# ktncktnc/diffusion-forcing-transformer

Hardware: AMD Instinct MI355X
Metric: denoised latent frames/sec, DFoT RE10K 8f & 200f rollout @1/2/4/8 GPU (higher is better)
Workload: dtype bf16

## Files before the change

### diffusion-forcing-transformer_amd/csrc/gemm.h

```cpp
#pragma once
#include "common.h"

namespace dfot {

enum AMode { A_DENSE = 0, A_CONV3 = 1, A_CONV3T = 2 };
enum Epi { E_F32 = 0, E_BF16 = 1, E_QKV = 2, E_QKV_DIT = 3 };

struct GemmArgs {
  const bf16* A = nullptr;
  long lda = 0;
  const bf16* W = nullptr;
  long ldw = 0;
  int M = 0, N = 0, K = 0;
  int H = 0, Wd = 0, Cin = 0;
  const bf16* zeros = nullptr;
  const uint8_t* live = nullptr;
  int To = 0, Tin = 0, Hin = 0, Win = 0;
  int cs = 1, ct = 1, ckt = 1;
  const float* bias = nullptr;
  float* out_f32 = nullptr;
  bf16* out_bf16 = nullptr;
  long ldo = 0;
  const float* resid = nullptr;
  const bf16* resid_bf = nullptr;
  const float* gate = nullptr;
  const int* gate_index = nullptr;
  long ldg = 0;
  int gate_rows = 0;
  int act = 0;
  bf16* pre_act = nullptr;
  bf16* raw = nullptr;
  long ldraw = 0;
  int bias_rows = 0;
  int tr_rows = 0;
  float* gn_part = nullptr;
  int gn_rows_per_bt = 0;
  int gn_cpg = 0;
  bf16* out2 = nullptr;
  long ldo2 = 0;
  int split = 0;
  bf16 *q = nullptr, *k = nullptr, *v = nullptr;
  const float *qw = nullptr, *kw = nullptr, *rope_cs = nullptr;
  int heads = 0, d = 0, ntok = 0;
  float qscale = 1.f;
  int dstride = 0;
  float eps = 1e-6f;
  int xcd = 1;
  int persist = 0;
  int ksplit = 1;
  long slice_stride = 0;
};

enum GemmVariant {
  GEMM_REGS_128 = 0,
  GEMM_DMA_128 = 1,
  GEMM_DMA_256x256 = 4,
  GEMM_DMA_512x128 = 6,
  GEMM_DMA_128_KS2 = 8,
  GEMM_DMA_256x192 = 9,
  GEMM_DMA_128x192 = 10,
  GEMM_DMA3_256x144 = 14,
  GEMM_AUTO = -1
};
int gemm_pick_variant(int amode, int m, int n, int k, bool plain_f32 = false);
int launch_gemm(int amode, int epi, int variant, const GemmArgs& g, hipStream_t stream);

}
```

### diffusion-forcing-transformer_amd/csrc/gemm.hip

```cpp
#include "gemm.h"
#include "dfot_hip.h"

namespace dfot {

constexpr int BK = 64;
constexpr int wave_cols(int bn) { return bn % 64 == 0 ? 64 : 48; }
constexpr int tile_threads(int bm, int bn, int wtm, int ks) { return (bm / wtm) * (bn / wave_cols(bn)) * 64 * ks; }
constexpr int EP_LD = 68;

template <int N>
__device__ __forceinline__ void wait_all_but() {
  static_assert(N == 2 || N == 4 || N == 6 || N == 8 || N == 12, "unexpected load count");
  if constexpr (N == 2) asm volatile("s_waitcnt vmcnt(2)\n\ts_barrier" ::: "memory");
  if constexpr (N == 4) asm volatile("s_waitcnt vmcnt(4)\n\ts_barrier" ::: "memory");
  if constexpr (N == 6) asm volatile("s_waitcnt vmcnt(6)\n\ts_barrier" ::: "memory");
  if constexpr (N == 8) asm volatile("s_waitcnt vmcnt(8)\n\ts_barrier" ::: "memory");
  if constexpr (N == 12) asm volatile("s_waitcnt vmcnt(12)\n\ts_barrier" ::: "memory");
}

__device__ __forceinline__ void wait_all_but_n(int n) {
  switch (n) {
    case 1: asm volatile("s_waitcnt vmcnt(1)\n\ts_barrier" ::: "memory"); break;
    case 2: asm volatile("s_waitcnt vmcnt(2)\n\ts_barrier" ::: "memory"); break;
    case 3: asm volatile("s_waitcnt vmcnt(3)\n\ts_barrier" ::: "memory"); break;
    case 4: asm volatile("s_waitcnt vmcnt(4)\n\ts_barrier" ::: "memory"); break;
    case 5: asm volatile("s_waitcnt vmcnt(5)\n\ts_barrier" ::: "memory"); break;
    case 6: asm volatile("s_waitcnt vmcnt(6)\n\ts_barrier" ::: "memory"); break;
    case 7: asm volatile("s_waitcnt vmcnt(7)\n\ts_barrier" ::: "memory"); break;
    case 8: asm volatile("s_waitcnt vmcnt(8)\n\ts_barrier" ::: "memory"); break;
    default: asm volatile("s_waitcnt vmcnt(0)\n\ts_barrier" ::: "memory"); break;
  }
}

template <int BM_T, int BN_T, int WTM, int NST, int AMODE, int EPI, bool DMA, int KS, int BKT>
__device__ __forceinline__ void gemm_tile(const GemmArgs& g, const int tile_index, const int tile_count) {
  static_assert(BKT == 64 || (BKT == 32 && AMODE == A_DENSE && DMA && KS == 1), "K-tile depth");
  constexpr int CPR = BKT / 8;
  constexpr int RPI = 64 / CPR;
  constexpr int ROWB = BKT * 2;
  constexpr int MI = WTM / 16;
  constexpr int WTN = wave_cols(BN_T);
  constexpr int NI = WTN / 16;
  constexpr int WN = BN_T / WTN;
  static_assert(WTN == 64 || (EPI == E_F32 || EPI == E_BF16), "48-column wave tiles: plain epilogues only");
  static_assert(WTN == 64 || KS == 1, "48-column wave tiles: no intra-workgroup split-K");
  constexpr int NW = (BM_T / WTM) * WN;
  constexpr int NT = NW * 64;
  constexpr int AINS = BM_T / RPI, WINS = BN_T / RPI;
  constexpr int ACH = (AINS + NW - 1) / NW;
  constexpr int WCH = (WINS + NW - 1) / NW;
  constexpr bool A_EVEN = AINS % NW == 0, W_EVEN = WINS % NW == 0;
  static_assert((A_EVEN && W_EVEN) || (DMA && KS == 1), "uneven staging: LDS-DMA kernels without intra-workgroup split-K only");
  constexpr int A_BYTES = BM_T * BKT * 2;
  constexpr int STAGE_BYTES = (BM_T + BN_T) * BKT * 2;
  constexpr int LOADS = ACH + WCH;
  static_assert(DMA || NST == 2, "register staging supports two stages only");
  static_assert(KS == 1 || (NST == 2 && DMA && EPI != E_QKV), "split-K: two-stage LDS-DMA kernels without in-epilogue barriers");
  extern __shared__ __attribute__((aligned(16))) char smem_all[];
  const int tid = threadIdx.x, lane = tid & 63;
  const int kgroup = KS == 1 ? 0 : (tid >> 6) / NW;
  const int wave = KS == 1 ? (tid >> 6) : (tid >> 6) % NW;
  char* smem = smem_all + kgroup * (NST * STAGE_BYTES);
  const int wm = wave / WN, wn = wave % WN;
  const int tiles_n = (g.N + BN_T - 1) / BN_T;
  const int ksplit = (EPI == E_F32 && (AMODE == A_DENSE || g.slice_stride > 0) && g.ksplit > 1) ? g.ksplit : 1;
  const int kslice = ksplit > 1 ? tile_index % ksplit : 0;
  const int bid = ksplit > 1 ? xcd_remap(tile_index / ksplit, tile_count / ksplit, g.xcd) : xcd_remap(tile_index, tile_count, g.xcd);
  const int tn = bid % tiles_n, tm = bid / tiles_n;
  const int m0 = tm * BM_T, n0 = tn * BN_T;
  if constexpr (AMODE == A_CONV3) {
    if (g.live && !g.live[(unsigned)m0 / (unsigned)(g.H * g.Wd)]) return;
  }
  int nk = g.K / BKT;
  long kbeg = 0;
  if (ksplit > 1) {
    const int per = nk / ksplit, rem = nk % ksplit;
    kbeg = (long)(kslice * per + (kslice < rem ? kslice : rem)) * BKT;
    nk = per + (kslice < rem ? 1 : 0);
  }
  auto swz = [](int r) { return BKT == 64 ? ((r >> 1) & 7) : ((r >> 2) & 2); };

  const int prow = lane / CPR;
  const int ppos = lane % CPR;
  const bf16* a_src[ACH];
  int a_y[ACH], a_x[ACH];
  [[maybe_unused]] int a_t[ACH];
  const bf16* w_src[WCH];
  int a_chunk[ACH];
#pragma unroll
  for (int i = 0; i < ACH; ++i) {
    const int r = RPI * (NW * i + wave) + prow;
    const int c = ppos ^ swz(r);
    a_chunk[i] = c;
    const long m = (long)m0 + r;
    if constexpr (AMODE == A_DENSE) {
      a_src[i] = g.A + m * g.lda + c * 8 + kbeg;
      a_y[i] = a_x[i] = 0;
    } else if constexpr (AMODE == A_CONV3) {
      const unsigned mu = (unsigned)m;
      const int xw = (int)(mu % (unsigned)g.Wd);
      const int yh = (int)((mu / (unsigned)g.Wd) % (unsigned)g.H);
      a_x[i] = xw;
      a_y[i] = yh;
      a_src[i] = g.A + m * (long)g.Cin + c * 8;
    } else {
      unsigned mu = (unsigned)m;
      const int xo = (int)(mu % (unsigned)g.Wd);
      mu /= (unsigned)g.Wd;
      const int yo = (int)(mu % (unsigned)g.H);
      mu /= (unsigned)g.H;
// ... 24 lines not shown
    cv_dx = tap % 3 - 1;
  } else if constexpr (AMODE == A_CONV3T) {
    const int kbase = kgroup * BKT + (int)kbeg;
    const int tap = kbase / g.Cin;
    cv_c0 = kbase - tap * g.Cin;
    cv_dt = tap / 9;
    cv_dy = (tap % 9) / 3;
    cv_dx = tap % 3;
  }
  auto a_addr = [&](int i, int kt) -> const bf16* {
    if constexpr (AMODE == A_DENSE) {
      return a_src[i] + (long)kt * BKT;
    } else if constexpr (AMODE == A_CONV3) {
      const int yy = a_y[i] + cv_dy, xx = a_x[i] + cv_dx;
      const bool ok = (yy >= 0) && (yy < g.H) && (xx >= 0) && (xx < g.Wd);
      const bf16* p = a_src[i] + ((long)cv_dy * g.Wd + cv_dx) * g.Cin + cv_c0;
      return ok ? p : g.zeros + a_chunk[i] * 8;
    } else {
      int tt = a_t[i] + cv_dt;
      tt = tt < 0 ? 0 : tt;
      const int yy = a_y[i] + cv_dy, xx = a_x[i] + cv_dx;
      const bool ok = (yy >= 0) && (yy < g.Hin) && (xx >= 0) && (xx < g.Win);
      const bf16* p = a_src[i] + ((long)(tt * g.Hin + yy) * g.Win + xx) * g.Cin + cv_c0;
      return ok ? p : g.zeros + a_chunk[i] * 8;
    }
  };
  auto conv_advance = [&]() {
    if constexpr (AMODE == A_CONV3) {
      cv_c0 += KS * BKT;
      while (cv_c0 >= g.Cin) {
        cv_c0 -= g.Cin;
        if (++cv_dx > 1) {
          cv_dx = -1;
          ++cv_dy;
        }
      }
    } else if constexpr (AMODE == A_CONV3T) {
      cv_c0 += KS * BKT;
      while (cv_c0 >= g.Cin) {
        cv_c0 -= g.Cin;
        if (++cv_dx > 2) {
          cv_dx = 0;
          if (++cv_dy > 2) {
            cv_dy = 0;
            ++cv_dt;
          }
        }
      }
    }
  };

  bf16x8 ra[ACH], rw[WCH];

  auto issue = [&](int kt, int stage) {
    char* sa = smem + stage * STAGE_BYTES;
    char* sw = sa + A_BYTES;
#pragma unroll
    for (int i = 0; i < ACH; ++i) {
      if (!A_EVEN && NW * i + wave >= AINS) continue;
      const bf16* pa = a_addr(i, kt);
      if constexpr (DMA) {
        __builtin_amdgcn_global_load_lds(DFOT_GLOBAL_PTR(pa), DFOT_LDS_PTR(sa + (NW * i + wave) * 1024), 16, 0, 0);
      } else {
        ra[i] = *reinterpret_cast<const bf16x8*>(pa);
      }
    }
#pragma unroll
    for (int i = 0; i < WCH; ++i) {
      if (!W_EVEN && NW * i + wave >= WINS) continue;
      const bf16* pw = w_src[i] + (long)kt * BKT;
      if constexpr (DMA) {
        __builtin_amdgcn_global_load_lds(DFOT_GLOBAL_PTR(pw), DFOT_LDS_PTR(sw + (NW * i + wave) * 1024), 16, 0, 0);
      } else {
        rw[i] = *reinterpret_cast<const bf16x8*>(pw);
      }
    }
    conv_advance();
  };
  auto commit = [&](int stage) {
    char* sa = smem + stage * STAGE_BYTES;
    char* sw = sa + A_BYTES;
#pragma unroll
    for (int i = 0; i < ACH; ++i) *reinterpret_cast<bf16x8*>(sa + (NW * i + wave) * 1024 + lane * 16) = ra[i];
#pragma unroll
    for (int i = 0; i < WCH; ++i) *reinterpret_cast<bf16x8*>(sw + (NW * i + wave) * 1024 + lane * 16) = rw[i];
  };

  f32x4 acc[MI][NI];
#pragma unroll
  for (int i = 0; i < MI; ++i)
#pragma unroll
    for (int j = 0; j < NI; ++j) acc[i][j] = f32x4{0.f, 0.f, 0.f, 0.f};

  const int frow = lane & 15, fk = lane >> 4;
  auto compute = [&](int stage) {
    const char* sa = smem + stage * STAGE_BYTES;
    const char* sw = sa + A_BYTES;
#pragma unroll
    for (int ks = 0; ks < BKT / 32; ++ks) {
      bf16x8 af[MI], wf[NI];
#pragma unroll
      for (int mi = 0; mi < MI; ++mi) {
        const int r = wm * WTM + mi * 16 + frow;
        const int pos = (ks * 4 + fk) ^ swz(r);
        af[mi] = *reinterpret_cast<const bf16x8*>(sa + r * ROWB + pos * 16);
      }
#pragma unroll
      for (int ni = 0; ni < NI; ++ni) {
        const int r = wn * WTN + ni * 16 + frow;
        const int pos = (ks * 4 + fk) ^ swz(r);
        wf[ni] = *reinterpret_cast<const bf16x8*>(sw + r * ROWB + pos * 16);
      }
#pragma unroll
      for (int mi = 0; mi < MI; ++mi)
#pragma unroll
        for (int ni = 0; ni < NI; ++ni)
          acc[mi][ni] = __builtin_amdgcn_mfma_f32_16x16x32_bf16(af[mi], wf[ni], acc[mi][ni], 0, 0, 0);
    }
  };

  if constexpr (NST == 2 && KS == 1) {
    issue(0, 0);
    if constexpr (DMA) {
      asm volatile("s_waitcnt vmcnt(0)" ::: "memory");
    } else {
      commit(0);
    }
    __syncthreads();
    for (int kt = 0; kt < nk; ++kt) {
      const int cur = kt & 1;
      if (kt + 1 < nk) issue(kt + 1, cur ^ 1);
      compute(cur);
      if constexpr (DMA) {
        asm volatile("s_waitcnt vmcnt(0)" ::: "memory");
      } else {
        if (kt + 1 < nk) commit(cur ^ 1);
      }
      __syncthreads();
    }
  } else if constexpr (NST == 2) {
    const int nit = (nk + KS - 1) / KS;
    if (kgroup < nk) issue(kgroup, 0);
    asm volatile("s_waitcnt vmcnt(0)" ::: "memory");
    __syncthreads();
    for (int it = 0; it < nit; ++it) {
      const int cur = it & 1;
      const int kt = it * KS + kgroup;
      if (kt + KS < nk) issue(kt + KS, cur ^ 1);
      if (kt < nk) compute(cur);
      asm volatile("s_waitcnt vmcnt(0)" ::: "memory");
      __syncthreads();
    }
    float* red = reinterpret_cast<float*>(smem_all) + wave * (MI * 16 * 64);
    if (kgroup == 1) {
#pragma unroll
      for (int mi = 0; mi < MI; ++mi)
#pragma unroll
        for (int ni = 0; ni < 4; ++ni)
#pragma unroll
          for (int j = 0; j < 4; ++j) red[((mi * 4 + ni) * 4 + j) * 64 + lane] = acc[mi][ni][j];
    }
    __syncthreads();
    if (kgroup == 1) return;
#pragma unroll
    for (int mi = 0; mi < MI; ++mi)
#pragma unroll
      for (int ni = 0; ni < 4; ++ni)
#pragma unroll
        for (int j = 0; j < 4; ++j) acc[mi][ni][j] += red[((mi * 4 + ni) * 4 + j) * 64 + lane];
  } else {
    static_assert(NST >= 3, "ring");
    [[maybe_unused]] const int my_loads =
        __builtin_amdgcn_readfirstlane((AINS - wave + NW - 1) / NW + (WINS - wave + NW - 1) / NW);
    auto ring_wait = [&]() {
      if constexpr (A_EVEN && W_EVEN) wait_all_but<(NST - 2) * LOADS>();
      else wait_all_but_n((NST - 2) * my_loads);
    };
#pragma unroll
    for (int t = 0; t < NST - 1; ++t)
      if (t < nk) issue(t, t);
    if (nk >= NST - 1) {
      ring_wait();
    } else {
      asm volatile("s_waitcnt vmcnt(0)\n\ts_barrier" ::: "memory");
    }
    int st = 0;
    for (int kt = 0; kt < nk; ++kt) {
      const int nxt = st == 0 ? NST - 1 : st - 1;
      if (kt + NST - 1 < nk) issue(kt + NST - 1, nxt);
      compute(st);
      if (kt + NST - 1 < nk) {
        ring_wait();
      } else {
        asm volatile("s_waitcnt vmcnt(0)\n\ts_barrier" ::: "memory");
      }
      st = st == NST - 1 ? 0 : st + 1;
    }
  }

  float* ep =reinterpret_cast<float*>(smem_all) + (KS == 2 ? NW * MI * 16 * 64 : 0) + wave * (16 * EP_LD);
  const int colq = lane & 15, rowq = (lane >> 4) * 4;
  const int nw = n0 + wn * WTN;
  [[maybe_unused]] const bool has_res = g.resid != nullptr;
  [[maybe_unused]] const bool has_gate = g.gate != nullptr;
  [[maybe_unused]] float gsum = 0.f, gsq = 0.f, gsum2 = 0.f, gsq2 = 0.f;
  const int cw = EPI == E_F32 ? (lane & 15) * 4 : (lane & 7) * 8;
  const int col = nw + cw;
  const bool live = col < g.N && cw < WTN;
  f32x4 b0 = {0.f, 0.f, 0.f, 0.f}, b1 = {0.f, 0.f, 0.f, 0.f};
  [[maybe_unused]] const bool bias2d = g.bias_rows != 0;
  [[maybe_unused]] const unsigned bias_den = (unsigned)(g.bias_rows > 0 ? g.bias_rows : -g.bias_rows);
  [[maybe_unused]] const bool bias_mod = g.bias_rows > 0;
  [[maybe_unused]] float bc[NI];
  if constexpr (EPI == E_QKV) {
#pragma unroll
    for (int ni = 0; ni < NI; ++ni) {
      const int c = nw + ni * 16 + colq;
      bc[ni] = (g.bias && c < g.N) ? g.bias[c] : 0.f;
    }
  } else if (g.bias && live && !bias2d && kslice == 0) {
    b0 = *reinterpret_cast<const f32x4*>(g.bias + col);
    if constexpr (EPI != E_F32) b1 = *reinterpret_cast<const f32x4*>(g.bias + col + 4);
  }
  if constexpr (EPI == E_BF16) {
    if (g.tr_rows > 0) {
#pragma unroll
      for (int mi = 0; mi < MI; ++mi) {
        const unsigned row = (unsigned)(m0 + wm * WTM + mi * 16 + rowq);
        const long frame = row / (unsigned)g.tr_rows;
        const int rin = (int)(row % (unsigned)g.tr_rows);
#pragma unroll
        for (int ni = 0; ni < NI; ++ni) {
          const int c = nw + ni * 16 + colq;
          if (c < g.N) {
            bf16x4 o;
#pragma unroll
            for (int j = 0; j < 4; ++j) o[j] = f2bf(acc[mi][ni][j]);
            *reinterpret_cast<bf16x4*>(g.out_bf16 + (frame * g.N + c) * (long)g.tr_rows + rin) = o;
          }
        }
      }
      return;
    }
  }
  [[maybe_unused]] f32x4 res_cur[4], gate_cur;
  [[maybe_unused]] const bool pre_gate = EPI == E_F32 && has_gate && live && g.gate_rows % 16 == 0;
  [[maybe_unused]] auto load_gate = [&](int mi) {
    long gr = (unsigned)(m0 + wm * WTM + mi * 16) / (unsigned)g.gate_rows;
    if (g.gate_index) gr = g.gate_index[gr];
// ... 310 lines not shown
          }
        }
      }
    }
  }

  if constexpr (EPI == E_F32 || EPI == E_BF16) {
    if (g.gn_part) {
      const unsigned mrow = (unsigned)(m0 + wm * WTM);
      const int bt = (int)(mrow / (unsigned)g.gn_rows_per_bt);
      const int slots = g.gn_rows_per_bt / 64;
      const int slot = (int)((mrow % (unsigned)g.gn_rows_per_bt) / 64);
      float* dst = g.gn_part + ((long)bt * slots + slot) * 64;
      if constexpr (EPI == E_F32) {
        if (g.gn_cpg == 8) {
          gsum += __shfl_xor(gsum, 1);
          gsq += __shfl_xor(gsq, 1);
        }
        gsum += __shfl_xor(gsum, 16);
        gsq += __shfl_xor(gsq, 16);
        gsum += __shfl_xor(gsum, 32);
        gsq += __shfl_xor(gsq, 32);
        if (lane < 16 && live && (g.gn_cpg == 4 || (lane & 1) == 0)) {
          const int grp = col / g.gn_cpg;
          dst[grp * 2] = gsum;
          dst[grp * 2 + 1] = gsq;
        }
      } else {
        if (g.gn_cpg == 8) {
          gsum += gsum2;
          gsq += gsq2;
        }
#pragma unroll
        for (int o = 8; o < 64; o <<= 1) {
          gsum += __shfl_xor(gsum, o);
          gsq += __shfl_xor(gsq, o);
          gsum2 += __shfl_xor(gsum2, o);
          gsq2 += __shfl_xor(gsq2, o);
        }
        if (lane < 8 && live) {
          const int grp = col / g.gn_cpg;
          dst[grp * 2] = gsum;
          dst[grp * 2 + 1] = gsq;
          if (g.gn_cpg == 4) {
            dst[grp * 2 + 2] = gsum2;
            dst[grp * 2 + 3] = gsq2;
          }
        }
      }
    }
  }
}

template <int BM_T, int BN_T, int WTM, int NST, int AMODE, int EPI, bool DMA, int KS = 1, int BKT = BK>
__global__ __launch_bounds__(tile_threads(BM_T, BN_T, WTM, KS)) void gemm_kernel(GemmArgs g) {
  gemm_tile<BM_T, BN_T, WTM, NST, AMODE, EPI, DMA, KS, BKT>(g, blockIdx.x, gridDim.x);
}

template <int BM_T, int BN_T, int WTM, int NST, int AMODE, int EPI, bool DMA, int KS = 1, int BKT = BK>
__global__ __launch_bounds__(tile_threads(BM_T, BN_T, WTM, KS)) void gemm_kernel_persistent(GemmArgs g, int tile_count) {
  for (int tile = blockIdx.x; tile < tile_count; tile += gridDim.x) {
    gemm_tile<BM_T, BN_T, WTM, NST, AMODE, EPI, DMA, KS, BKT>(g, tile, tile_count);
    if (tile + (int)gridDim.x < tile_count) __syncthreads();
  }
}

template <int BM_T, int BN_T, int WTM, int NST, int AMODE, int EPI, bool DMA, int KS = 1, int BKT = BK>
static int launch_t(const GemmArgs& g, hipStream_t stream) {
  constexpr int nthreads = tile_threads(BM_T, BN_T, WTM, KS);
  constexpr int stage_lds = KS * NST * (BM_T + BN_T) * BKT * 2;
  constexpr int ep_lds = (nthreads / 64) * 16 * EP_LD * 4 + 2 * (nthreads / 64) * 16 * 4 +
                         (KS == 2 ? (nthreads / 128) * (WTM / 16) * 16 * 64 * 4 : 0);
  constexpr int lds = stage_lds > ep_lds ? stage_lds : ep_lds;
  const int ksplit = (EPI == E_F32 && (AMODE == A_DENSE || g.slice_stride > 0) && g.ksplit > 1) ? g.ksplit : 1;
  const int tiles = (g.M / BM_T) * ((g.N + BN_T - 1) / BN_T) * ksplit;
  GemmArgs ga = g;
  ga.xcd = 1;
  ga.persist = 1;
  constexpr bool kPersistOK = KS == 1 && nthreads <= 768;
  if constexpr (kPersistOK) {
    if (ga.persist > 0 && ksplit == 1) {
      const int resident = 256 * (lds <= 80 * 1024 ? 2 : 1);
      if (tiles > resident) {
        auto kp = gemm_kernel_persistent<BM_T, BN_T, WTM, NST, AMODE, EPI, DMA, KS, BKT>;
        static bool pattr_set = false;
        if (!pattr_set) {
          DFOT_CHECK_HIP(hipFuncSetAttribute(reinterpret_cast<const void*>(kp), hipFuncAttributeMaxDynamicSharedMemorySize, lds));
          pattr_set = true;
        }
        hipLaunchKernelGGL(kp, dim3(resident), dim3(nthreads), lds, stream, ga, tiles);
        DFOT_CHECK_HIP(hipGetLastError());
        return DFOT_OK;
      }
    }
  }
  auto kern = gemm_kernel<BM_T, BN_T, WTM, NST, AMODE, EPI, DMA, KS, BKT>;
  static bool attr_set = false;
  if (!attr_set) {
    DFOT_CHECK_HIP(hipFuncSetAttribute(reinterpret_cast<const void*>(kern), hipFuncAttributeMaxDynamicSharedMemorySize, lds));
    attr_set = true;
  }
  hipLaunchKernelGGL(kern, dim3(tiles), dim3(nthreads), lds, stream, ga);
  DFOT_CHECK_HIP(hipGetLastError());
  return DFOT_OK;
}

template <int AMODE, int EPI>
static int launch_v(int variant, const GemmArgs& g, hipStream_t s) {
  switch (variant) {
    case GEMM_REGS_128:
      if constexpr (AMODE == A_CONV3T) break;
      else return launch_t<128, 128, 64, 2, AMODE, EPI, false>(g, s);
    case GEMM_DMA_128: return launch_t<128, 128, 64, 2, AMODE, EPI, true>(g, s);
    case GEMM_DMA_256x256: return launch_t<256, 256, 64, 2, AMODE, EPI, true>(g, s);
    case GEMM_DMA_512x128: return launch_t<512, 128, 64, 2, AMODE, EPI, true>(g, s);
    case GEMM_DMA_256x192:
      if constexpr (AMODE != A_DENSE) break;
      else return launch_t<256, 192, 64, 2, AMODE, EPI, true>(g, s);
    case GEMM_DMA3_256x144:
      if constexpr ((EPI != E_F32 && !(EPI == E_BF16 && AMODE == A_DENSE)) || AMODE == A_CONV3T) break;
      else {
        if (g.gn_part) break;
        return launch_t<256, 144, 64, 3, AMODE, EPI, true>(g, s);
      }
    case GEMM_DMA_128x192:
      if constexpr (AMODE != A_DENSE || EPI == E_QKV) break;
      else return launch_t<128, 192, 64, 2, AMODE, EPI, true>(g, s);
    case GEMM_DMA_128_KS2:
      if constexpr (EPI == E_QKV) break;
      else return launch_t<128, 128, 64, 2, AMODE, EPI, true, 2>(g, s);
  }
  set_error("gemm: unknown variant %d", variant);
  return DFOT_ERR_ARG;
}

int gemm_pick_variant(int amode, int m, int n, int k, bool plain_f32) {
  const long tiles = (long)(m / 256) * ((n + 255) / 256);
  if (m % 256 == 0 && n >= 192 && amode == A_DENSE) {
    auto util = [&](int bn) {
      const long t = (long)(m / 256) * ((n + bn - 1) / bn);
      return (double)m * n / ((double)((t + 255) / 256) * 256 * 256 * bn);
    };
    if (plain_f32 && n % 144 == 0 && k >= 2304 && (long)(m / 256) * (n / 144) >= 256 && util(144) > 1.1 * util(192) && util(144) > 1.1 * util(256))
      return GEMM_DMA3_256x144;
    if (util(192) > 1.05 * util(256) && (long)(m / 256) * ((n + 191) / 192) >= 160) return GEMM_DMA_256x192;
  }
  if (m % 256 == 0 && n >= 192 && tiles >= 160) return GEMM_DMA_256x256;
  if (m % 512 == 0 && n <= 128 && m / 512 >= 256) return GEMM_DMA_512x128;
  const long tiles128 = (long)(m / 128) * ((n + 127) / 128);
  if (tiles128 <= 256 && k >= 2048) return GEMM_DMA_128_KS2;
  return GEMM_DMA_128;
}

int launch_gemm(int amode, int epi, int variant, const GemmArgs& g, hipStream_t stream) {
  DFOT_REQUIRE(g.A && g.W, DFOT_ERR_ARG, "gemm: null operand");
  if (variant == GEMM_AUTO) variant = gemm_pick_variant(amode, g.M, g.N, g.K, epi == E_F32 && !g.gn_part);
  if (variant == GEMM_DMA_128_KS2 && epi == E_QKV) variant = GEMM_DMA_128;
  if (variant == GEMM_DMA_128x192 && epi == E_QKV) variant = GEMM_DMA_128;
  if (variant == GEMM_DMA_256x192 && epi == E_QKV && g.d != 64) variant = GEMM_DMA_256x256;
  const int bm = variant == GEMM_DMA_512x128 ? 512 : (variant == GEMM_DMA_256x256 || variant == GEMM_DMA_256x192 || variant == GEMM_DMA3_256x144) ? 256 : 128;
  DFOT_REQUIRE(g.M > 0 && g.M % bm == 0, DFOT_ERR_SHAPE, "gemm: M=%d must be a positive multiple of %d", g.M, bm);
  DFOT_REQUIRE(g.K > 0 && g.K % BK == 0, DFOT_ERR_SHAPE, "gemm: K=%d must be a positive multiple of %d", g.K, BK);
  DFOT_REQUIRE(g.N > 0 && g.N % (epi == E_F32 ? 4 : 8) == 0, DFOT_ERR_SHAPE, "gemm: N=%d must be a multiple of %d", g.N, epi == E_F32 ? 4 : 8);
  DFOT_REQUIRE((epi == E_QKV || epi == E_QKV_DIT || g.ldo % (epi == E_F32 ? 4 : 8) == 0) && (epi != E_QKV || (g.ldo2 % 8 == 0 && g.split % 64 == 0)),
               DFOT_ERR_SHAPE, "gemm: output row strides must be multiples of %d", epi == E_F32 ? 4 : 8);
  DFOT_REQUIRE(g.ldw == 0 || (amode == A_DENSE && g.ldw >= g.K && g.ldw % 8 == 0), DFOT_ERR_SHAPE, "gemm: ldw=%ld must be >= K and a multiple of 8 (dense A only)", g.ldw);
  if (amode == A_CONV3) {
    DFOT_REQUIRE(g.Cin % BK == 0 && g.K == 9 * g.Cin, DFOT_ERR_SHAPE, "conv3x3: Cin=%d must be a multiple of %d", g.Cin, BK);
    DFOT_REQUIRE(g.zeros != nullptr, DFOT_ERR_ARG, "conv3x3: zero page missing");
    DFOT_REQUIRE(g.H > 0 && g.Wd > 0 && g.M % (g.H * g.Wd) == 0, DFOT_ERR_SHAPE, "conv3x3: M=%d not a whole number of %dx%d images", g.M, g.H, g.Wd);
    DFOT_REQUIRE(!g.live || (g.H * g.Wd) % bm == 0, DFOT_ERR_SHAPE, "conv3x3: live-image flags need whole %d-row tiles per %dx%d image", bm, g.H, g.Wd);
  }
  if (amode == A_CONV3T) {
    DFOT_REQUIRE(epi == E_F32 && g.ksplit <= 1 && !g.live && !g.gate && !g.bias_rows, DFOT_ERR_ARG, "conv3t: plain fp32 epilogue only");
    DFOT_REQUIRE(g.Cin % BK == 0 && (g.ckt == 1 || g.ckt == 3) && g.K == g.ckt * 9 * g.Cin && (g.cs == 1 || g.cs == 2) && (g.ct == 1 || g.ct == 2),
                 DFOT_ERR_SHAPE, "conv3t: Cin=%d (multiple of %d), kt=%d in {1,3}, K=%d = kt*9*Cin, strides s=%d t=%d in {1,2}", g.Cin, BK, g.ckt, g.K,
                 g.cs, g.ct);
    DFOT_REQUIRE(g.zeros != nullptr, DFOT_ERR_ARG, "conv3t: zero page missing");
    DFOT_REQUIRE(g.H > 0 && g.Wd > 0 && g.To > 0 && g.Hin == g.cs * g.H && g.Win == g.cs * g.Wd && g.Tin >= 1 && g.ct * (g.To - 1) <= g.Tin - 1 &&
                     g.To == (g.Tin - 1) / g.ct + 1,
                 DFOT_ERR_SHAPE, "conv3t: input %dx%dx%d, output %dx%dx%d do not match strides s=%d t=%d", g.Tin, g.Hin, g.Win, g.To, g.H, g.Wd, g.cs, g.ct);
    DFOT_REQUIRE(g.M % (g.To * g.H * g.Wd) == 0, DFOT_ERR_SHAPE, "conv3t: M=%d not a whole number of %dx%dx%d videos", g.M, g.To, g.H, g.Wd);
    DFOT_REQUIRE((long)g.Tin * g.Hin * g.Win * g.Cin < (1L << 31), DFOT_ERR_SHAPE, "conv3t: one input video must hold < 2^31 elements");
  }
  if (epi == E_QKV) {
    DFOT_REQUIRE(g.q && g.k && g.v && g.qw && g.kw && g.rope_cs && (g.out2 || g.N == g.split), DFOT_ERR_ARG, "qkv epilogue: null pointer");
    DFOT_REQUIRE(!g.raw || (g.ldraw >= g.N && g.ldraw % 8 == 0), DFOT_ERR_SHAPE, "qkv epilogue: raw copy needs ldraw >= N, a multiple of 8");
    DFOT_REQUIRE((g.d == 64 || g.d == 128) && g.heads > 0 && g.split == 3 * g.heads * g.d && g.ntok > 0 && g.M % g.ntok == 0,
                 DFOT_ERR_SHAPE, "qkv epilogue: heads=%d d=%d split=%d ntok=%d M=%d", g.heads, g.d, g.split, g.ntok, g.M);
  }
  if (epi == E_QKV_DIT) {
    DFOT_REQUIRE(g.q && g.k && g.v, DFOT_ERR_ARG, "dit qkv epilogue: null pointer");
    DFOT_REQUIRE(g.d > 0 && g.d % 8 == 0 && g.dstride >= g.d && g.dstride % 8 == 0 && g.heads > 0 && g.N == 3 * g.heads * g.d &&
                     g.ntok > 0 && g.M % g.ntok == 0,
                 DFOT_ERR_SHAPE, "dit qkv epilogue: heads=%d d=%d dstride=%d ntok=%d M=%d N=%d", g.heads, g.d, g.dstride, g.ntok, g.M, g.N);
  }
  if (g.gate) {
    DFOT_REQUIRE(epi == E_F32 && g.gate_rows > 0 && g.M % g.gate_rows == 0 && g.ldg % 4 == 0, DFOT_ERR_SHAPE,
                 "gemm: gate needs the fp32 epilogue, gate_rows dividing M and ldg %% 4 == 0");
  }
  if (g.ksplit > 1 && g.slice_stride > 0)
    DFOT_REQUIRE(!g.bias && !g.resid, DFOT_ERR_ARG, "gemm: split-K into partial outputs takes no bias / residual");
  if (g.ksplit > 1)
    DFOT_REQUIRE(epi == E_F32 && (amode == A_DENSE || g.slice_stride > 0) && !g.bias_rows && (!g.resid || g.resid == g.out_f32) && !g.gate &&
                     !g.gn_part && g.K / BK >= 2 * g.ksplit, DFOT_ERR_ARG,
                 "gemm: split-K over workgroups needs the fp32 epilogue with an in-place residual (or none), no gate, and K >= %d", 2 * g.ksplit * BK);
  if (g.bias_rows) DFOT_REQUIRE((epi == E_F32 || epi == E_BF16) && g.bias, DFOT_ERR_ARG, "gemm: 2-D bias needs a plain epilogue");
  if (g.resid_bf)
    DFOT_REQUIRE(epi == E_BF16 && (amode == A_CONV3 || variant == GEMM_DMA3_256x144) && !g.resid, DFOT_ERR_ARG,
                 "gemm: a bf16 residual needs the bf16 epilogue of a convolution or of the 256x144 ring");
  if (g.tr_rows) {
    DFOT_REQUIRE(epi == E_BF16 && !g.bias && !g.act && !g.gn_part && g.tr_rows % 4 == 0 && g.M % g.tr_rows == 0 && amode == A_DENSE,
                 DFOT_ERR_ARG, "gemm: transposed store needs the plain bf16 epilogue and tr_rows %% 4 == 0 dividing M");
  }
  if (g.gn_part) {
    DFOT_REQUIRE(epi != E_QKV && epi != E_QKV_DIT && (g.gn_cpg == 4 || g.gn_cpg == 8) && g.N == 32 * g.gn_cpg && g.gn_rows_per_bt % 64 == 0 &&
                     g.gn_rows_per_bt % bm == 0,
                 DFOT_ERR_SHAPE, "gemm: fused GroupNorm statistics need N = 32 groups of 4 or 8 channels and whole images per tile");
  }
  if (amode == A_DENSE) {
    switch (epi) {
      case E_F32: return launch_v<A_DENSE, E_F32>(variant, g, stream);
      case E_BF16: return launch_v<A_DENSE, E_BF16>(variant, g, stream);
      case E_QKV: return launch_v<A_DENSE, E_QKV>(variant, g, stream);
      case E_QKV_DIT: return launch_v<A_DENSE, E_QKV_DIT>(variant, g, stream);
    }
  } else if (amode == A_CONV3) {
    switch (epi) {
      case E_F32: return launch_v<A_CONV3, E_F32>(variant, g, stream);
      case E_BF16: return launch_v<A_CONV3, E_BF16>(variant, g, stream);
    }
  } else if (amode == A_CONV3T && epi == E_F32) {
    return launch_v<A_CONV3T, E_F32>(variant, g, stream);
  }
  set_error("gemm: unsupported mode/epilogue combination %d/%d", amode, epi);
  return DFOT_ERR_ARG;
}

}
```

### diffusion-forcing-transformer_amd/csrc/uvit.hip

```cpp
#include <algorithm>
#include <cmath>
#include <cstdarg>
#include <cstdlib>
#include <cstring>
#include <functional>
#include <map>
#include <string>
#include <vector>

#include "dfot_hip.h"
#include "gemm.h"
#include "kernels.h"

namespace dfot {

static thread_local char g_err[1024] = "";
void set_error(const char* fmt, ...) {
  va_list ap;
  va_start(ap, fmt);
  vsnprintf(g_err, sizeof(g_err), fmt, ap);
  va_end(ap);
}
const char* get_error() { return g_err; }

// ... 370 lines not shown
  const long i = (long)blockIdx.x * blockDim.x + threadIdx.x;
  if (i >= total4) return;
  const f4 b = reinterpret_cast<const f4*>(y)[i];
  const bf16x4 xv = reinterpret_cast<const bf16x4*>(x)[i];
  reinterpret_cast<bf16x4*>(x)[i] = bf16x4{f2bf(bf2f(xv[0]) + b[0]), f2bf(bf2f(xv[1]) + b[1]), f2bf(bf2f(xv[2]) + b[2]), f2bf(bf2f(xv[3]) + b[3])};
}

static void swap_out_part(dfot_uvit_s* h) { h->pend_part = h->out_part; }

static int flush_pending(dfot_uvit_s* h, hipStream_t s) {
  if (!h->pend_bias) return DFOT_OK;
  const long total4 = h->pend_m * h->pend_c / 4;
  hipLaunchKernelGGL(out_reduce_kernel, dim3(cdiv(total4, 256)), dim3(256), 0, s, h->XB[h->pend_lvl], h->pend_bias, h->pend_part,
                     h->pend_part + h->pend_m * h->pend_c, h->pend_slices == 3 ? h->pend_part + 2 * h->pend_m * h->pend_c : nullptr, total4,
                     h->pend_c / 4);
  h->pend_bias = nullptr;
  DFOT_CHECK_HIP(hipGetLastError());
  return DFOT_OK;
}

static int run_tr_block(dfot_uvit_s* h, const TrW& w, int lvl, int batch, hipStream_t s) {
  const int c = w.c, rr = h->r[lvl], n = h->T * rr * rr, d = c / h->heads;
  const int m = batch * n;
  bf16* xb = h->XB[lvl];
  int rc = 0;
  if (h->pend_bias && (h->pend_lvl != lvl || h->pend_m != m || h->pend_c != c) && (rc = flush_pending(h, s))) return rc;
  if (!h->xin_bf[lvl]) {
    if ((rc = launch_f32_to_bf16(h->xin[lvl], xb, (long)m * c, s))) return rc;
    h->xin_bf[lvl] = true;
  }
  RmsPending pend{xb, h->pend_bias, h->pend_part, h->pend_part + (long)m * c, h->pend_slices == 3 ? h->pend_part + 2L * m * c : nullptr};
  if ((rc = launch_rms_film_bf16(xb, w.nw, w.fcache, h->sv + w.sv_off, h->have_mask ? h->cond_mask : nullptr, h->s1, m, c, rr * rr, h->T,
                                 h->cfg.eps, s, h->pend_bias ? &pend : nullptr)))
    return rc;
  h->pend_bias = nullptr;
  GemmArgs p;
  p.A = h->s1; p.lda = c; p.W = w.w_fused; p.M = m; p.N = 7 * c; p.K = c; p.bias = w.b_fused;
  p.out2 = h->cat + c; p.ldo2 = 5 * c; p.split = 3 * c;
  p.q = h->q; p.k = h->k; p.v = h->v; p.qw = w.qw; p.kw = w.kw; p.rope_cs = h->rope_cs[lvl]; p.heads = h->heads; p.d = d;
  p.ntok = n; p.qscale = 1.4426950408889634f / sqrtf((float)d); p.eps = h->cfg.eps;
  if ((rc = launch_gemm(A_DENSE, E_QKV, h->gemm_variant, p, s))) return rc;
  const bool timed = h->time_attn && lvl == 2 && h->ev_used < h->ev_start.size();
  if (timed) DFOT_CHECK_HIP(hipEventRecord(h->ev_start[h->ev_used], s));
  int av = h->attn_variant;
  if (av == 2 && d == 64 && n % 256 == 0) av = (w.score_bound < 64.0f && !h->attn_force_safe) ? 14 : 5;
  if ((rc = launch_attention(h->q, h->k, h->v, h->cat, 5 * c, batch, h->heads, n, d, av, s, &h->attn_scratch))) return rc;
  if (timed) DFOT_CHECK_HIP(hipEventRecord(h->ev_stop[h->ev_used++], s));
  GemmArgs o;
  o.A = h->cat; o.lda = 5 * c; o.W = w.w_out; o.M = m; o.N = c; o.K = 5 * c; o.bias = w.b_out; o.ldo = c;
  if (h->gemm_variant == GEMM_AUTO && h->out_part && (size_t)2 * m * c <= h->out_part_elems && m % 256 == 0 && c % 144 == 0 &&
      (long)(m / 256) * (c / 144) * 2 <= 256 && (5 * c / 64) >= 8) {
    GemmArgs p2 = o;
    p2.bias = nullptr; p2.out_f32 = h->out_part; p2.ksplit = 2; p2.slice_stride = (long)m * c;
    if ((rc = launch_gemm(A_DENSE, E_F32, GEMM_DMA3_256x144, p2, s))) return rc;
    h->pend_bias = w.b_out;
    h->pend_lvl = lvl; h->pend_m = m; h->pend_c = c; h->pend_slices = 2;
    swap_out_part(h);
    return DFOT_OK;
  }
  if (h->gemm_variant == GEMM_AUTO && c % 144 == 0 && m % 256 == 0 && (long)(m / 256) * ((c + 191) / 192) < 256 &&
      (long)(m / 256) * (c / 144) >= 200 && (long)(m / 256) * (c / 144) <= 256) {
    o.out_bf16 = xb;
    o.resid_bf = xb;
    return launch_gemm(A_DENSE, E_BF16, GEMM_DMA3_256x144, o, s);
  }
  o.out_f32 = h->X[lvl];
  if ((rc = launch_gemm(A_DENSE, E_F32, h->gemm_variant, o, s))) return rc;
  hipLaunchKernelGGL(add_f32_into_bf16_kernel, dim3(cdiv((long)m * c / 4, 256)), dim3(256), 0, s, xb, h->X[lvl], (long)m * c / 4);
  DFOT_CHECK_HIP(hipGetLastError());
  return DFOT_OK;
}


__global__ void slab_reduce_kernel(float* __restrict__ out, const float* __restrict__ bias, const float* __restrict__ slabs, int nslab, long stride4,
                                   long total4, int cq, const uint8_t* __restrict__ live, unsigned img4) {
  typedef __attribute__((ext_vector_type(4))) float f4;
  const long i = (long)blockIdx.x * blockDim.x + threadIdx.x;
  if (i >= total4) return;
  if (live && !live[(unsigned)i / img4]) return;
  f4 v = reinterpret_cast<const f4*>(bias)[i % cq];
  for (int sl = 0; sl < nslab; ++sl) v += reinterpret_cast<const f4*>(slabs)[sl * stride4 + i];
  reinterpret_cast<f4*>(out)[i] = v;
}

static int conv_between_levels(dfot_uvit_s* h, GemmArgs g, hipStream_t s) {
  const long px = (long)g.H * g.Wd;
  if (h->gemm_variant == GEMM_AUTO && h->out_part && !g.gn_part && g.M % 256 == 0 && px % 256 == 0 && (g.N % 144 == 0 || g.N == 256) &&
      (long)g.M * g.N < (1L << 31)) {
    const int bn = g.N % 144 == 0 ? 144 : 256;
    const int variant = bn == 144 ? GEMM_DMA3_256x144 : GEMM_DMA_256x256;
    const int tiles = (g.M / 256) * (g.N / bn);
    int ks = 1;
    while (tiles * ks * 2 <= 256 && g.K / 64 / (ks * 2) >= 16) ks *= 2;
    if (tiles * ks >= 192 && tiles * ks <= 256) {
      if (ks == 1) return launch_gemm(A_CONV3, E_F32, variant, g, s);
      if ((size_t)ks * g.M * g.N <= h->out_part_elems) {
        GemmArgs p = g;
        float* out = g.out_f32;
        const float* bias = g.bias;
        p.bias = nullptr; p.resid = nullptr; p.out_f32 = h->out_part; p.ksplit = ks; p.slice_stride = (long)g.M * g.N;
        int rc = launch_gemm(A_CONV3, E_F32, variant, p, s);
        if (rc) return rc;
        const long total4 = (long)g.M * g.N / 4;
        hipLaunchKernelGGL(slab_reduce_kernel, dim3(cdiv(total4, 256)), dim3(256), 0, s, out, bias, h->out_part, ks, total4, total4, g.N / 4, g.live,
                           (unsigned)(px * g.N / 4));
        DFOT_CHECK_HIP(hipGetLastError());
        return DFOT_OK;
      }
    }
  }
  return launch_gemm(A_CONV3, E_F32, h->gemm_variant, g, s);
}

static int run_down(dfot_uvit_s* h, int l, int bt, hipStream_t s, const uint8_t* live = nullptr) {
  const int rr = h->r[l], cin = h->ch[l], cout = h->ch[l + 1];
  int rc = 0;
  if ((rc = h->xin_bf[l] ? launch_pool2_bf16_bf16in(h->XB[l], h->s1, bt, rr, rr, cin, s) : launch_pool2_bf16(h->xin[l], h->s1, bt, rr, rr, cin, s)))
    return rc;
  GemmArgs g;
  g.A = h->s1; g.W = h->down_conv[l].w; g.M = bt * (rr / 2) * (rr / 2); g.N = cout; g.K = 9 * cin; g.H = rr / 2; g.Wd = rr / 2;
  g.Cin = cin; g.zeros = h->zeros; g.bias = h->down_conv[l].b; g.out_f32 = h->HSA[l]; g.ldo = cout;
  g.live = live;
  const bool next_is_res = l + 1 < 2;
  if (next_is_res) {
    g.gn_part = h->gn_partial; g.gn_rows_per_bt = (rr / 2) * (rr / 2); g.gn_cpg = cout / 32;
  }
  if ((rc = conv_between_levels(h, g, s))) return rc;
  h->gn1_nblk = next_is_res ? g.gn_rows_per_bt / 64 : 0;
  h->xin[l + 1] = h->HSA[l];
  h->xin_bf[l + 1] = false;
  return DFOT_OK;
}

static int run_up(dfot_uvit_s* h, int l, int bt, hipStream_t s, const uint8_t* live = nullptr) {
  const int rr = h->r[l + 1], cin = h->ch[l + 1], cout = h->ch[l];
  const long n_in = (long)bt * rr * rr * cin;
  int rc = 0;
  if ((rc = h->xin_bf[l + 1] ? launch_sub_bf16_bf16in(h->XB[l + 1], h->HSA[l], h->s1, n_in, s, live, (long)rr * rr * cin)
                             : launch_sub_bf16(h->xin[l + 1], h->HSA[l], h->s1, n_in, s, live, (long)rr * rr * cin)))
    return rc;
  GemmArgs g;
  g.A = h->s1; g.W = h->up_conv[l].w; g.M = bt * rr * rr; g.N = cout; g.K = 9 * cin; g.H = rr; g.Wd = rr; g.Cin = cin;
  g.zeros = h->zeros; g.bias = h->up_conv[l].b; g.out_f32 = h->tmp; g.ldo = cout;
// ... 510 lines not shown
```

Baseline: 9.943.

## Add software-scheduled 256x144 ring GEMM variant with fine-grained LDS waits

Adds a SCHED=1 path for the 3-stage 256x144 LDS-DMA GEMM. All LDS fragment reads for a K-tile are issued up front, and per-row lgkmcnt waits let MFMAs start as soon as their operands arrive. The main loop is specialised on compile-time per-wave load counts, so vmcnt waits are exact for uneven staging. The attention out-projection and the between-level conv GEMMs now use this variant. The cost is higher register pressure from holding all fragments at once, and the persistent-kernel path is disabled for it.

```diff
diff --git a/diffusion-forcing-transformer_amd/csrc/gemm.h b/diffusion-forcing-transformer_amd/csrc/gemm.h
--- a/diffusion-forcing-transformer_amd/csrc/gemm.h
+++ b/diffusion-forcing-transformer_amd/csrc/gemm.h
@@ -60,6 +60,7 @@
   GEMM_DMA_256x192 = 9,
   GEMM_DMA_128x192 = 10,
   GEMM_DMA3_256x144 = 14,
+  GEMM_DMA3_256x144_PF = 15,
   GEMM_AUTO = -1
 };
 int gemm_pick_variant(int amode, int m, int n, int k, bool plain_f32 = false);
diff --git a/diffusion-forcing-transformer_amd/csrc/gemm.hip b/diffusion-forcing-transformer_amd/csrc/gemm.hip
--- a/diffusion-forcing-transformer_amd/csrc/gemm.hip
+++ b/diffusion-forcing-transformer_amd/csrc/gemm.hip
@@ -1,5 +1,7 @@
 #include "gemm.h"
 #include "dfot_hip.h"
+
+#include <type_traits>
 
 namespace dfot {
 
@@ -10,8 +12,11 @@
 
 template <int N>
 __device__ __forceinline__ void wait_all_but() {
-  static_assert(N == 2 || N == 4 || N == 6 || N == 8 || N == 12, "unexpected load count");
+  static_assert((N >= 1 && N <= 6) || N == 8 || N == 12, "unexpected load count");
+  if constexpr (N == 1) asm volatile("s_waitcnt vmcnt(1)\n\ts_barrier" ::: "memory");
   if constexpr (N == 2) asm volatile("s_waitcnt vmcnt(2)\n\ts_barrier" ::: "memory");
+  if constexpr (N == 3) asm volatile("s_waitcnt vmcnt(3)\n\ts_barrier" ::: "memory");
+  if constexpr (N == 5) asm volatile("s_waitcnt vmcnt(5)\n\ts_barrier" ::: "memory");
   if constexpr (N == 4) asm volatile("s_waitcnt vmcnt(4)\n\ts_barrier" ::: "memory");
   if constexpr (N == 6) asm volatile("s_waitcnt vmcnt(6)\n\ts_barrier" ::: "memory");
   if constexpr (N == 8) asm volatile("s_waitcnt vmcnt(8)\n\ts_barrier" ::: "memory");
@@ -32,7 +37,28 @@
   }
 }
 
-template <int BM_T, int BN_T, int WTM, int NST, int AMODE, int EPI, bool DMA, int KS, int BKT>
+__device__ __forceinline__ void lgkm_wait(int n) {
+  switch (n) {
+    case 0: asm volatile("s_waitcnt lgkmcnt(0)" ::: "memory"); break;
+    case 1: asm volatile("s_waitcnt lgkmcnt(1)" ::: "memory"); break;
+    case 2: asm volatile("s_waitcnt lgkmcnt(2)" ::: "memory"); break;
+    case 3: asm volatile("s_waitcnt lgkmcnt(3)" ::: "memory"); break;
+    case 4: asm volatile("s_waitcnt lgkmcnt(4)" ::: "memory"); break;
+    case 5: asm volatile("s_waitcnt lgkmcnt(5)" ::: "memory"); break;
+    case 6: asm volatile("s_waitcnt lgkmcnt(6)" ::: "memory"); break;
+    case 7: asm volatile("s_waitcnt lgkmcnt(7)" ::: "memory"); break;
+    case 8: asm volatile("s_waitcnt lgkmcnt(8)" ::: "memory"); break;
+    case 9: asm volatile("s_waitcnt lgkmcnt(9)" ::: "memory"); break;
+    case 10: asm volatile("s_waitcnt lgkmcnt(10)" ::: "memory"); break;
+    case 11: asm volatile("s_waitcnt lgkmcnt(11)" ::: "memory"); break;
+    case 12: asm volatile("s_waitcnt lgkmcnt(12)" ::: "memory"); break;
+    case 13: asm volatile("s_waitcnt lgkmcnt(13)" ::: "memory"); break;
+    case 14: asm volatile("s_waitcnt lgkmcnt(14)" ::: "memory"); break;
+    default: break;
+  }
+}
+
+template <int BM_T, int BN_T, int WTM, int NST, int AMODE, int EPI, bool DMA, int KS, int BKT, int SCHED>
 __device__ __forceinline__ void gemm_tile(const GemmArgs& g, const int tile_index, const int tile_count) {
   static_assert(BKT == 64 || (BKT == 32 && AMODE == A_DENSE && DMA && KS == 1), "K-tile depth");
   constexpr int CPR = BKT / 8;
@@ -56,6 +82,7 @@
   constexpr int LOADS = ACH + WCH;
   static_assert(DMA || NST == 2, "register staging supports two stages only");
   static_assert(KS == 1 || (NST == 2 && DMA && EPI != E_QKV), "split-K: two-stage LDS-DMA kernels without in-epilogue barriers");
+  static_assert(SCHED == 0 || (NST >= 3 && KS == 1), "SCHED = 1: ring kernels only");
   extern __shared__ __attribute__((aligned(16))) char smem_all[];
   const int tid = threadIdx.x, lane = tid & 63;
   const int kgroup = KS == 1 ? 0 : (tid >> 6) / NW;
@@ -186,12 +213,13 @@
 
   bf16x8 ra[ACH], rw[WCH];
 
-  auto issue = [&](int kt, int stage) {
+  auto issue_c = [&](int kt, int stage, auto na_c, auto nw_c) {
+    constexpr int NA = decltype(na_c)::value, NWL = decltype(nw_c)::value;
     char* sa = smem + stage * STAGE_BYTES;
     char* sw = sa + A_BYTES;
 #pragma unroll
     for (int i = 0; i < ACH; ++i) {
-      if (!A_EVEN && NW * i + wave >= AINS) continue;
+      if (NA >= 0 ? i >= NA : (!A_EVEN && NW * i + wave >= AINS)) continue;
       const bf16* pa = a_addr(i, kt);
       if constexpr (DMA) {
         __builtin_amdgcn_global_load_lds(DFOT_GLOBAL_PTR(pa), DFOT_LDS_PTR(sa + (NW * i + wave) * 1024), 16, 0, 0);
@@ -201,7 +229,7 @@
     }
 #pragma unroll
     for (int i = 0; i < WCH; ++i) {
-      if (!W_EVEN && NW * i + wave >= WINS) continue;
+      if (NWL >= 0 ? i >= NWL : (!W_EVEN && NW * i + wave >= WINS)) continue;
       const bf16* pw = w_src[i] + (long)kt * BKT;
       if constexpr (DMA) {
         __builtin_amdgcn_global_load_lds(DFOT_GLOBAL_PTR(pw), DFOT_LDS_PTR(sw + (NW * i + wave) * 1024), 16, 0, 0);
@@ -211,6 +239,7 @@
     }
     conv_advance();
   };
+  auto issue = [&](int kt, int stage) { issue_c(kt, stage, std::integral_constant<int, -1>{}, std::integral_constant<int, -1>{}); };
   auto commit = [&](int stage) {
     char* sa = smem + stage * STAGE_BYTES;
     char* sw = sa + A_BYTES;
@@ -230,6 +259,37 @@
   auto compute = [&](int stage) {
     const char* sa = smem + stage * STAGE_BYTES;
     const char* sw = sa + A_BYTES;
+    if constexpr (SCHED == 1) {
+      constexpr int NR = NI + MI, KSN = BKT / 32;
+      static_assert(KSN * NR <= 15, "lgkmcnt counts at most 15 reads");
+      bf16x8 af[KSN][MI], wf[KSN][NI];
+      const unsigned la = (unsigned)(uintptr_t)DFOT_LDS_PTR(sa), lw = (unsigned)(uintptr_t)DFOT_LDS_PTR(sw);
+#pragma unroll
+      for (int ks = 0; ks < KSN; ++ks) {
+#pragma unroll
+        for (int ni = 0; ni < NI; ++ni) {
+          const int r = wn * WTN + ni * 16 + frow;
+          asm volatile("ds_read_b128 %0, %1" : "=v"(wf[ks][ni]) : "v"(lw + r * ROWB + ((ks * 4 + fk) ^ swz(r)) * 16));
+        }
+#pragma unroll
+        for (int mi = 0; mi < MI; ++mi) {
+          const int r = wm * WTM + mi * 16 + frow;
+          asm volatile("ds_read_b128 %0, %1" : "=v"(af[ks][mi]) : "v"(la + r * ROWB + ((ks * 4 + fk) ^ swz(r)) * 16));
+        }
+      }
+#pragma unroll
+      for (int ks = 0; ks < KSN; ++ks)
+#pragma unroll
+        for (int mi = 0; mi < MI; ++mi) {
+          const int after = (MI - 1 - mi) + (KSN - 1 - ks) * NR;
+          lgkm_wait(after);
+          __builtin_amdgcn_sched_barrier(0);
+#pragma unroll
+          for (int ni = 0; ni < NI; ++ni)
+            acc[mi][ni] = __builtin_amdgcn_mfma_f32_16x16x32_bf16(af[ks][mi], wf[ks][ni], acc[mi][ni], 0, 0, 0);
+        }
+      return;
+    }
 #pragma unroll
     for (int ks = 0; ks < BKT / 32; ++ks) {
       bf16x8 af[MI], wf[NI];
@@ -310,6 +370,44 @@
       if constexpr (A_EVEN && W_EVEN) wait_all_but<(NST - 2) * LOADS>();
       else wait_all_but_n((NST - 2) * my_loads);
     };
+    if constexpr (SCHED == 1) {
+      auto ring = [&](auto na_c, auto nw_c) {
+        constexpr int NA = decltype(na_c)::value, NWL = decltype(nw_c)::value;
+#pragma unroll
+        for (int t = 0; t < NST - 1; ++t)
+          if (t < nk) issue_c(t, t, na_c, nw_c);
+        if (nk >= NST - 1) {
+          wait_all_but<(NST - 2) * (NA + NWL)>();
+        } else {
+          asm volatile("s_waitcnt vmcnt(0)\n\ts_barrier" ::: "memory");
+        }
+        int st = 0;
+        for (int kt = 0; kt < nk; ++kt) {
+          const int nxt = st == 0 ? NST - 1 : st - 1;
+          if (kt + NST - 1 < nk) issue_c(kt + NST - 1, nxt, na_c, nw_c);
+          compute(st);
+          if (kt + NST - 1 < nk) {
+            wait_all_but<(NST - 2) * (NA + NWL)>();
+          } else {
+            asm volatile("s_waitcnt vmcnt(0)\n\ts_barrier" ::: "memory");
+          }
+          st = st == NST - 1 ? 0 : st + 1;
+        }
+      };
+      using A1 = std::integral_constant<int, ACH>;
+      using A0 = std::integral_constant<int, A_EVEN ? ACH : ACH - 1>;
+      using W1 = std::integral_constant<int, WCH>;
+      using W0 = std::integral_constant<int, W_EVEN ? WCH : WCH - 1>;
+      const bool full_a = __builtin_amdgcn_readfirstlane(NW * (ACH - 1) + wave < AINS);
+      const bool full_w = __builtin_amdgcn_readfirstlane(NW * (WCH - 1) + wave < WINS);
+      if (full_a) {
+        if (full_w) ring(A1{}, W1{});
+        else ring(A1{}, W0{});
+      } else {
+        if (full_w) ring(A0{}, W1{});
+        else ring(A0{}, W0{});
+      }
+    } else {
 #pragma unroll
     for (int t = 0; t < NST - 1; ++t)
       if (t < nk) issue(t, t);
@@ -329,6 +427,7 @@
         asm volatile("s_waitcnt vmcnt(0)\n\ts_barrier" ::: "memory");
       }
       st = st == NST - 1 ? 0 : st + 1;
+    }
     }
   }
 
@@ -745,20 +844,20 @@
   }
 }
 
-template <int BM_T, int BN_T, int WTM, int NST, int AMODE, int EPI, bool DMA, int KS = 1, int BKT = BK>
+template <int BM_T, int BN_T, int WTM, int NST, int AMODE, int EPI, bool DMA, int KS = 1, int BKT = BK, int SCHED = 0>
 __global__ __launch_bounds__(tile_threads(BM_T, BN_T, WTM, KS)) void gemm_kernel(GemmArgs g) {
-  gemm_tile<BM_T, BN_T, WTM, NST, AMODE, EPI, DMA, KS, BKT>(g, blockIdx.x, gridDim.x);
+  gemm_tile<BM_T, BN_T, WTM, NST, AMODE, EPI, DMA, KS, BKT, SCHED>(g, blockIdx.x, gridDim.x);
 }
 
-template <int BM_T, int BN_T, int WTM, int NST, int AMODE, int EPI, bool DMA, int KS = 1, int BKT = BK>
+template <int BM_T, int BN_T, int WTM, int NST, int AMODE, int EPI, bool DMA, int KS = 1, int BKT = BK, int SCHED = 0>
 __global__ __launch_bounds__(tile_threads(BM_T, BN_T, WTM, KS)) void gemm_kernel_persistent(GemmArgs g, int tile_count) {
   for (int tile = blockIdx.x; tile < tile_count; tile += gridDim.x) {
-    gemm_tile<BM_T, BN_T, WTM, NST, AMODE, EPI, DMA, KS, BKT>(g, tile, tile_count);
+    gemm_tile<BM_T, BN_T, WTM, NST, AMODE, EPI, DMA, KS, BKT, SCHED>(g, tile, tile_count);
     if (tile + (int)gridDim.x < tile_count) __syncthreads();
   }
 }
 
-template <int BM_T, int BN_T, int WTM, int NST, int AMODE, int EPI, bool DMA, int KS = 1, int BKT = BK>
+template <int BM_T, int BN_T, int WTM, int NST, int AMODE, int EPI, bool DMA, int KS = 1, int BKT = BK, int SCHED = 0>
 static int launch_t(const GemmArgs& g, hipStream_t stream) {
   constexpr int nthreads = tile_threads(BM_T, BN_T, WTM, KS);
   constexpr int stage_lds = KS * NST * (BM_T + BN_T) * BKT * 2;
@@ -770,12 +869,12 @@
   GemmArgs ga = g;
   ga.xcd = 1;
   ga.persist = 1;
-  constexpr bool kPersistOK = KS == 1 && nthreads <= 768;
+  constexpr bool kPersistOK = KS == 1 && nthreads <= 768 && SCHED == 0;
   if constexpr (kPersistOK) {
     if (ga.persist > 0 && ksplit == 1) {
       const int resident = 256 * (lds <= 80 * 1024 ? 2 : 1);
       if (tiles > resident) {
-        auto kp = gemm_kernel_persistent<BM_T, BN_T, WTM, NST, AMODE, EPI, DMA, KS, BKT>;
+        auto kp = gemm_kernel_persistent<BM_T, BN_T, WTM, NST, AMODE, EPI, DMA, KS, BKT, SCHED>;
         static bool pattr_set = false;
         if (!pattr_set) {
           DFOT_CHECK_HIP(hipFuncSetAttribute(reinterpret_cast<const void*>(kp), hipFuncAttributeMaxDynamicSharedMemorySize, lds));
@@ -787,7 +886,7 @@
       }
     }
   }
-  auto kern = gemm_kernel<BM_T, BN_T, WTM, NST, AMODE, EPI, DMA, KS, BKT>;
+  auto kern = gemm_kernel<BM_T, BN_T, WTM, NST, AMODE, EPI, DMA, KS, BKT, SCHED>;
   static bool attr_set = false;
   if (!attr_set) {
     DFOT_CHECK_HIP(hipFuncSetAttribute(reinterpret_cast<const void*>(kern), hipFuncAttributeMaxDynamicSharedMemorySize, lds));
@@ -816,6 +915,12 @@
         if (g.gn_part) break;
         return launch_t<256, 144, 64, 3, AMODE, EPI, true>(g, s);
       }
+    case GEMM_DMA3_256x144_PF:
+      if constexpr ((EPI != E_F32 && !(EPI == E_BF16 && AMODE == A_DENSE)) || AMODE == A_CONV3T) break;
+      else {
+        if (g.gn_part) break;
+        return launch_t<256, 144, 64, 3, AMODE, EPI, true, 1, BK, 1>(g, s);
+      }
     case GEMM_DMA_128x192:
       if constexpr (AMODE != A_DENSE || EPI == E_QKV) break;
       else return launch_t<128, 192, 64, 2, AMODE, EPI, true>(g, s);
@@ -851,7 +956,7 @@
   if (variant == GEMM_DMA_128_KS2 && epi == E_QKV) variant = GEMM_DMA_128;
   if (variant == GEMM_DMA_128x192 && epi == E_QKV) variant = GEMM_DMA_128;
   if (variant == GEMM_DMA_256x192 && epi == E_QKV && g.d != 64) variant = GEMM_DMA_256x256;
-  const int bm = variant == GEMM_DMA_512x128 ? 512 : (variant == GEMM_DMA_256x256 || variant == GEMM_DMA_256x192 || variant == GEMM_DMA3_256x144) ? 256 : 128;
+  const int bm = variant == GEMM_DMA_512x128 ? 512 : (variant == GEMM_DMA_256x256 || variant == GEMM_DMA_256x192 || variant == GEMM_DMA3_256x144 || variant == GEMM_DMA3_256x144_PF) ? 256 : 128;
   DFOT_REQUIRE(g.M > 0 && g.M % bm == 0, DFOT_ERR_SHAPE, "gemm: M=%d must be a positive multiple of %d", g.M, bm);
   DFOT_REQUIRE(g.K > 0 && g.K % BK == 0, DFOT_ERR_SHAPE, "gemm: K=%d must be a positive multiple of %d", g.K, BK);
   DFOT_REQUIRE(g.N > 0 && g.N % (epi == E_F32 ? 4 : 8) == 0, DFOT_ERR_SHAPE, "gemm: N=%d must be a multiple of %d", g.N, epi == E_F32 ? 4 : 8);
@@ -900,7 +1005,7 @@
                  "gemm: split-K over workgroups needs the fp32 epilogue with an in-place residual (or none), no gate, and K >= %d", 2 * g.ksplit * BK);
   if (g.bias_rows) DFOT_REQUIRE((epi == E_F32 || epi == E_BF16) && g.bias, DFOT_ERR_ARG, "gemm: 2-D bias needs a plain epilogue");
   if (g.resid_bf)
-    DFOT_REQUIRE(epi == E_BF16 && (amode == A_CONV3 || variant == GEMM_DMA3_256x144) && !g.resid, DFOT_ERR_ARG,
+    DFOT_REQUIRE(epi == E_BF16 && (amode == A_CONV3 || variant == GEMM_DMA3_256x144 || variant == GEMM_DMA3_256x144_PF) && !g.resid, DFOT_ERR_ARG,
                  "gemm: a bf16 residual needs the bf16 epilogue of a convolution or of the 256x144 ring");
   if (g.tr_rows) {
     DFOT_REQUIRE(epi == E_BF16 && !g.bias && !g.act && !g.gn_part && g.tr_rows % 4 == 0 && g.M % g.tr_rows == 0 && amode == A_DENSE,
diff --git a/diffusion-forcing-transformer_amd/csrc/uvit.hip b/diffusion-forcing-transformer_amd/csrc/uvit.hip
--- a/diffusion-forcing-transformer_amd/csrc/uvit.hip
+++ b/diffusion-forcing-transformer_amd/csrc/uvit.hip
@@ -446,7 +446,7 @@
       (long)(m / 256) * (c / 144) * 2 <= 256 && (5 * c / 64) >= 8) {
     GemmArgs p2 = o;
     p2.bias = nullptr; p2.out_f32 = h->out_part; p2.ksplit = 2; p2.slice_stride = (long)m * c;
-    if ((rc = launch_gemm(A_DENSE, E_F32, GEMM_DMA3_256x144, p2, s))) return rc;
+    if ((rc = launch_gemm(A_DENSE, E_F32, GEMM_DMA3_256x144_PF, p2, s))) return rc;
     h->pend_bias = w.b_out;
     h->pend_lvl = lvl; h->pend_m = m; h->pend_c = c; h->pend_slices = 2;
     swap_out_part(h);
@@ -456,7 +456,7 @@
       (long)(m / 256) * (c / 144) >= 200 && (long)(m / 256) * (c / 144) <= 256) {
     o.out_bf16 = xb;
     o.resid_bf = xb;
-    return launch_gemm(A_DENSE, E_BF16, GEMM_DMA3_256x144, o, s);
+    return launch_gemm(A_DENSE, E_BF16, GEMM_DMA3_256x144_PF, o, s);
   }
   o.out_f32 = h->X[lvl];
   if ((rc = launch_gemm(A_DENSE, E_F32, h->gemm_variant, o, s))) return rc;
@@ -482,7 +482,7 @@
   if (h->gemm_variant == GEMM_AUTO && h->out_part && !g.gn_part && g.M % 256 == 0 && px % 256 == 0 && (g.N % 144 == 0 || g.N == 256) &&
       (long)g.M * g.N < (1L << 31)) {
     const int bn = g.N % 144 == 0 ? 144 : 256;
-    const int variant = bn == 144 ? GEMM_DMA3_256x144 : GEMM_DMA_256x256;
+    const int variant = bn == 144 ? GEMM_DMA3_256x144_PF : GEMM_DMA_256x256;
     const int tiles = (g.M / 256) * (g.N / bn);
     int ks = 1;
     while (tiles * ks * 2 <= 256 && g.K / 64 / (ks * 2) >= 16) ks *= 2;
```

Result: faster. 10.07, median of 6 (+1.3%).
